# Luca96/carla-driving-rl-agent

Measured on AMD Instinct MI355X. Metric: PPO update-steps/sec (batch=256, 4x90x120x3 obs), higher is better.
Workload: dtype f32; 1 GPU; configs[1]: synthetic rollout buffer 256x4-frame 90x120x3 obs per GPU, full CARLANetwork fwd/bwd + PPO (re-sampled Beta, pathwise) / value loss + clip + Adam, fp32; per_gpu_batch=256, global_batch=256, parallelism=dp1, policy_loss=resampled (reference-faithful)

## Files before the change

### carla-driving-rl-agent_amd/csrc/gemm_pw_bwd.hip

```cpp
#include <stdlib.h>

#include "colreduce.h"

namespace cdrl {

typedef float f32x16 __attribute__((ext_vector_type(16)));
typedef __bf16 bf16x8 __attribute__((ext_vector_type(8)));
typedef __bf16 bf16x4 __attribute__((ext_vector_type(4)));
typedef uint32_t u32x2 __attribute__((ext_vector_type(2)));
typedef float f32x2 __attribute__((ext_vector_type(2)));

struct PwbArgs {
    View dz;
    int dz_shuffle;
    int act;
    const float* y;
    const float* stats;
    const float* coef;
    View a;
    const float* a_stats;
    const __bf16* Wp;
    int wp_ks;
    View da;
    float* qpart;
// ... 721 lines not shown
                    qacc[j] = __builtin_amdgcn_mfma_f32_32x32x16_bf16(a1, d1, qacc[j], 0, 0, 0);
                }
            }
        };
        if (t0 < t1) {
#pragma unroll
            for (int j = 0; j < 4; ++j) load_row(t0, j);
        }
        __syncthreads();
        for (int t = t0; t < t1; ++t) {
            store_tile(t);
            __syncthreads();
            compute_tile();
            __syncthreads();
        }
        float* qp = a.qpart + ((int64_t)g * a.nbpg + b) * KP * NP;
#pragma unroll
        for (int j = 0; j < NTW; ++j) {
            const int n = (qnt0 + j) * 32 + lrow;
#pragma unroll
            for (int r = 0; r < 16; ++r) {
                const int k = qkt * 32 + (r & 3) + 8 * (r >> 2) + 4 * lk;
                qp[k * NP + n] = qacc[j][r];
            }
        }
        __syncthreads();
        if (ANORM && a.spart) {
            __syncthreads();
            __syncthreads();
        }
    }
}

struct PwbReduceArgs {
    const float* qpart;
    const double* dbpart;
    const double* spart;
    const float* W;
    const float* a_stats;
    const float* a_gamma;
    const float* a_beta;
    float* dW;
    float* db;
    float* a_dgamma;
    float* a_dbeta;
    float* a_coef;
    const double* fin_tot;
    float* o_dgamma;
    float* o_dbeta;
    int N, K, KP, NP, G, Mg, nbpg;
    int wbf;
};

constexpr int PWB_RS = 8;
__global__ void __launch_bounds__(128 * PWB_RS) pwb_reduce_kernel(PwbReduceArgs a) {
    __shared__ double sq[PWB_RS][128];
    __shared__ double sd[PWB_RS][128];
    __shared__ double red[2][8][2];
    const int k = blockIdx.x, n = threadIdx.x & 127, sl = threadIdx.x >> 7;
    const int N = a.N, K = a.K, G = a.G;
    const bool on = n < N;
    const int nsl = PWB_RS / G > 0 ? PWB_RS / G : 1;
    const int per = (a.nbpg + nsl - 1) / nsl;
    for (int pair = sl; pair < G * nsl; pair += PWB_RS) {
        const int g = pair % G, s = pair / G;
        const int b0 = s * per, b1 = min(a.nbpg, b0 + per);
        double q = 0.0, d = 0.0;
        if (on) {
            const float* pq = a.qpart + ((int64_t)g * a.nbpg * a.KP + k) * a.NP + n;
            const double* pd = a.dbpart + (int64_t)g * a.nbpg * a.NP + n;
            int b = b0;
            const bool need_d = a.a_stats != nullptr || k == 0;
            for (; b + 32 <= b1; b += 32) {
                float v[32];
                double u[32];
#pragma unroll
                for (int i = 0; i < 32; ++i) {
                    v[i] = pq[(int64_t)(b + i) * a.KP * a.NP];
                    u[i] = need_d ? pd[(int64_t)(b + i) * a.NP] : 0.0;
                }
#pragma unroll
                for (int i = 0; i < 32; ++i) {
                    q += (double)v[i];
                    d += u[i];
                }
            }
            for (; b + 16 <= b1; b += 16) {
                float v[16];
                double u[16];
#pragma unroll
                for (int i = 0; i < 16; ++i) {
                    v[i] = pq[(int64_t)(b + i) * a.KP * a.NP];
                    u[i] = pd[(int64_t)(b + i) * a.NP];
                }
#pragma unroll
                for (int i = 0; i < 16; ++i) {
                    q += (double)v[i];
                    d += u[i];
                }
            }
            for (; b + 8 <= b1; b += 8) {
                float v[8];
                double u[8];
#pragma unroll
                for (int i = 0; i < 8; ++i) {
                    v[i] = pq[(int64_t)(b + i) * a.KP * a.NP];
                    u[i] = pd[(int64_t)(b + i) * a.NP];
                }
#pragma unroll
                for (int i = 0; i < 8; ++i) {
                    q += (double)v[i];
                    d += u[i];
                }
            }
            for (; b < b1; ++b) {
                q += (double)pq[(int64_t)b * a.KP * a.NP];
                d += pd[(int64_t)b * a.NP];
            }
        }
        sq[pair][n] = q;
        sd[pair][n] = d;
    }
    __syncthreads();
    const bool lead = sl == 0;
    float w = (on && lead) ? a.W[(int64_t)k * N + n] : 0.0f;
    if (a.wbf) w = (float)(__bf16)w;
    double qtot = 0.0, dbtot = 0.0;
    double s1[8], s2[8];
#pragma unroll
    for (int g = 0; g < 8; ++g) {
        s1[g] = s2[g] = 0.0;
        if (g < G && lead) {
            double q = sq[g][n], d = sd[g][n];
            for (int s = 1; s < nsl; ++s) {
                q += sq[s * G + g][n];
                d += sd[s * G + g][n];
            }
            qtot += q;
            dbtot += d;
            s1[g] = (double)w * d;
            s2[g] = (double)w * q;
        }
    }
    if (on && lead) {
        if (a.a_stats) a.dW[(int64_t)k * N + n] = (float)((double)a.a_gamma[k] * qtot + (double)a.a_beta[k] * dbtot);
        else a.dW[(int64_t)k * N + n] = (float)qtot;
        if (k == 0) a.db[n] = (float)dbtot;
        if (k == 0 && a.fin_tot) {
            double dg = 0.0, dbt = 0.0;
            for (int g = 0; g < G; ++g) {
                dbt += a.fin_tot[((int64_t)g * 2 + 0) * N + n];
                dg += a.fin_tot[((int64_t)g * 2 + 1) * N + n];
            }
            a.o_dgamma[n] = (float)dg;
            a.o_dbeta[n] = (float)dbt;
        }
    }
    if (!a.a_stats) return;
    const int lane = n & 63, wave = n >> 6;
#pragma unroll
    for (int g = 0; g < 8; ++g) {
        if (g >= G) break;
        double u1 = s1[g], u2 = s2[g];
#pragma unroll
        for (int o = 32; o > 0; o >>= 1) {
            u1 += __shfl_down(u1, o);
            u2 += __shfl_down(u2, o);
        }
        if (lane == 0 && lead) {
            red[0][g][wave] = u1;
            red[1][g][wave] = u2;
        }
    }
    __syncthreads();
    if (a.spart && (int)(threadIdx.x >> 6) < 2 * G) {
        const int pr = threadIdx.x >> 6, g = pr >> 1, q = pr & 1, l = threadIdx.x & 63;
        double u = 0.0;
        for (int b = l; b < a.nbpg; b += 64) u += a.spart[(((int64_t)g * a.nbpg + b) * 2 + q) * a.KP + k];
#pragma unroll
        for (int o = 32; o > 0; o >>= 1) u += __shfl_down(u, o);
        if (l == 0) {
            red[q][g][0] = u;
            red[q][g][1] = 0.0;
        }
    }
    __syncthreads();
    if (threadIdx.x == 0) {
        const int GK = G * K;
        const double cnt = (double)a.Mg;
        double dg = 0.0, dbt = 0.0;
        for (int g = 0; g < G; ++g) {
            const double u1 = red[0][g][0] + red[0][g][1], u2 = red[1][g][0] + red[1][g][1];
            dbt += u1;
            dg += u2;
            a.a_coef[0 * GK + g * K + k] = a.a_stats[2 * GK + g * K + k];
            a.a_coef[1 * GK + g * K + k] = (float)(u1 / cnt);
            a.a_coef[2 * GK + g * K + k] = (float)(u2 / cnt);
        }
        a.a_dgamma[k] = (float)dg;
        a.a_dbeta[k] = (float)dbt;
    }
}

static inline int pwb_pad(int c) { return c <= 64 ? 64 : 128; }

bool pw_bwd_fused_supported(View dz, View a, View da, int N, int K, int at) {
    if (N > 128 || K > 128 || N < 8 || K < 8 || (N & 1) || (K & 1)) return false;
    if (at && pwb_pad(N) != pwb_pad(K)) return false;
    if (pwb_pad(N) != pwb_pad(K) && !(pwb_pad(K) == 64 && pwb_pad(N) == 128)) return false;
    auto ok = [](View v) { return (v.ld % 2 == 0) && (v.coff % 2 == 0) && ((reinterpret_cast<uintptr_t>(v.p) & 7) == 0); };
    return ok(a) && ok(da) && (dz.ld % 2 == 0) && ((reinterpret_cast<uintptr_t>(dz.p) & 7) == 0);
}

int pw_bwd_fused_nbpg(int G, int Mg, int N, int K, int at) {
    const int bm = (pwb_pad(K) == 128 || pwb_pad(N) == 128) ? 32 : 64;
    const int tiles = cdiv(Mg, bm);
    int nb = 256 / G;
    if (at && tiles >= 6 * (512 / G)) nb = 512 / G;
    if (nb < 1) nb = 1;
    return nb > tiles ? tiles : nb;
}

int64_t pw_bwd_fused_qpart_elems(int G, int Mg, int N, int K, int at) {
    return (int64_t)G * pw_bwd_fused_nbpg(G, Mg, N, K, at) * pwb_pad(K) * pwb_pad(N);
}

int64_t pw_bwd_fused_dbpart_elems(int G, int Mg, int N, int K, int at) {
    return (int64_t)G * pw_bwd_fused_nbpg(G, Mg, N, K, at) * pwb_pad(N) * (at ? 3 : 1);
}

template <int KP, int NP, bool SHUF, bool ANORM, bool ACC>
static int pwb_launch(const PwbArgs& a, hipStream_t st) {
    constexpr int BM = (KP == 128 || NP == 128) ? 32 : 64;
    constexpr size_t lds = (size_t)(3 * BM * (NP + 8) + 3 * (NP + KP) * (BM + 8)) * 2 + (size_t)7 * NP * sizeof(float);
    auto kern = pwb_kernel<KP, NP, SHUF, ANORM, ACC>;
    static LdsAttrOnce attr;
    if (attr.need()) {
        CDRL_HIP(hipFuncSetAttribute(reinterpret_cast<const void*>(kern), hipFuncAttributeMaxDynamicSharedMemorySize, (int)lds));
        attr.mark();
    }
    hipLaunchKernelGGL(kern, dim3(a.G * a.nbpg), dim3(512), lds, st, a);
    CDRL_LAUNCH_CHECK();
    return 0;
}

template <int P, bool SHUF, bool ANORM, bool ACC>
static int pwb16_launch(const PwbArgs& a, hipStream_t st) {
    constexpr int BM = P == 128 ? 32 : 64;
    constexpr size_t lds = (size_t)(BM * (P + 8) + 2 * P * (BM + 8)) * 2 + (size_t)7 * P * sizeof(float) + (size_t)(P / 16) * 2 * 128 * 8 * 2;
    auto kern = pwb16_kernel<P, P, SHUF, ANORM, ACC>;
    static LdsAttrOnce attr;
    if (attr.need() && lds >= 64 * 1024) {
        CDRL_HIP(hipFuncSetAttribute(reinterpret_cast<const void*>(kern), hipFuncAttributeMaxDynamicSharedMemorySize, (int)lds));
// ... 62 lines not shown
        set_error("pw_bwd_fused: finalize-on-load needs the float32 form, fin_tot and fin_nb");
        return -1;
    }
    a.spart = (f.at && f.a_stats) ? f.dbpart + (int64_t)f.G * a.nbpg * pwb_pad(f.N) : nullptr;
    static const int dbg = cdrl_getenv("CDRL_DIAG_PWB") ? atoi(cdrl_getenv("CDRL_DIAG_PWB")) : 0;
    a.dbg = dbg;
    const bool anorm = f.a_stats != nullptr, acc = f.accumulate != 0, shuf = f.dz_shuffle != 0;
    if (f.at && pwb_pad(f.K) != pwb_pad(f.N)) {
        set_error("pw_bwd_fused: the bf16-storage form is instantiated for equal paddings only (N=%d K=%d)", f.N, f.K);
        return -1;
    }
    if (f.at) {
        if (pwb_pad(f.K) == 128) return shuf ? pwb16_launch2<128, true>(a, anorm, acc, st) : pwb16_launch2<128, false>(a, anorm, acc, st);
        return shuf ? pwb16_launch2<64, true>(a, anorm, acc, st) : pwb16_launch2<64, false>(a, anorm, acc, st);
    }
    if (pwb_pad(f.K) == 128) return shuf ? pwb_launch2<128, 128, true>(a, anorm, acc, st) : pwb_launch2<128, 128, false>(a, anorm, acc, st);
    if (pwb_pad(f.N) == 128) return shuf ? pwb_launch2<64, 128, true>(a, anorm, acc, st) : pwb_launch2<64, 128, false>(a, anorm, acc, st);
    return shuf ? pwb_launch2<64, 64, true>(a, anorm, acc, st) : pwb_launch2<64, 64, false>(a, anorm, acc, st);
}

int pw_bwd_fused_reduce(const PwBwdFused& f, hipStream_t st) {
    PwbReduceArgs r;
    r.qpart = f.qpart;
    r.dbpart = f.dbpart;
    r.W = f.W;
    r.a_stats = f.a_stats;
    r.a_gamma = f.a_gamma;
    r.a_beta = f.a_beta;
    r.dW = f.dW;
    r.db = f.db;
    r.a_dgamma = f.a_dgamma;
    r.a_dbeta = f.a_dbeta;
    r.a_coef = f.a_coef;
    r.N = f.N;
    r.K = f.K;
    r.KP = pwb_pad(f.K);
    r.NP = pwb_pad(f.N);
    r.G = f.G;
    r.Mg = f.Mg;
    r.nbpg = pw_bwd_fused_nbpg(f.G, f.Mg, f.N, f.K, f.at);
    r.wbf = f.at;
    r.fin_tot = (f.fin_part && !f.at) ? f.fin_tot : nullptr;
    r.o_dgamma = f.o_dgamma;
    r.o_dbeta = f.o_dbeta;
    if (r.fin_tot && (!f.o_dgamma || !f.o_dbeta)) {
        set_error("pw_bwd_fused_reduce: finalize-on-load needs the dgamma / dbeta outputs of the BatchNorm behind the conv");
        return -1;
    }
    r.spart = (f.at && f.a_stats) ? f.dbpart + (int64_t)f.G * r.nbpg * pwb_pad(f.N) : nullptr;
    if (f.a_stats && (!f.a_gamma || !f.a_beta || !f.a_dgamma || !f.a_dbeta || !f.a_coef)) {
        set_error("pw_bwd_fused_reduce: normalised input needs gamma / beta and the dgamma / dbeta / coef outputs");
        return -1;
    }
    hipLaunchKernelGGL(pwb_reduce_kernel, dim3(f.K), dim3(128 * PWB_RS), 0, st, r);
    CDRL_LAUNCH_CHECK();
    return 0;
}

}
```

### carla-driving-rl-agent_amd/csrc/gemm_pw_x3.hip

```cpp
#include <stdlib.h>

#include "cdrl_kernels.h"
#include "pack_bodies.h"

namespace cdrl {

typedef float f32x16 __attribute__((ext_vector_type(16)));
typedef __bf16 bf16x8 __attribute__((ext_vector_type(8)));
typedef __bf16 bf16x4 __attribute__((ext_vector_type(4)));

struct PwX3Args {
    View A;
    const float* pro_stats;
    const __bf16* Wp;
    const float* bias;
    View C;
    double* part;
    int N, K, G, Mg, nbpg;
};

__device__ __forceinline__ void split3(float x, __bf16& h1, __bf16& h2, __bf16& h3) {
    h1 = (__bf16)x;
    const float r1 = x - (float)h1;
    h2 = (__bf16)r1;
    h3 = (__bf16)(r1 - (float)h2);
}

template <int KP, int NT, bool PRO, bool EPI>
__global__ void __launch_bounds__(256, 2) pw_x3_kernel(PwX3Args a) {
    constexpr int WC = NT, WR = 4 / WC, BM = 32 * WR, KS = KP / 16;
    constexpr int LDA = KP + 8;
    constexpr int CPR = KP / 4;
    constexpr int NCH = BM * CPR / 256;
    __shared__ __attribute__((aligned(16))) __bf16 As[3][BM * LDA];
    __shared__ float pc[2][KP];
    __shared__ double red[2][4][32];
    const int tid = threadIdx.x, lane = tid & 63, wave = tid >> 6;
    const int wr = wave % WR, wc = wave / WR;
    const int lrow = lane & 31, lk = lane >> 5;
    const int g = blockIdx.x / a.nbpg, b = blockIdx.x % a.nbpg;
    const int K = a.K, N = a.N;
    const int64_t mbeg = (int64_t)g * a.Mg, mend = mbeg + a.Mg;
    const int tiles_g = (a.Mg + BM - 1) / BM;
    const int t0 = (int)((int64_t)b * tiles_g / a.nbpg), t1 = (int)((int64_t)(b + 1) * tiles_g / a.nbpg);
    const int n = wc * 32 + lrow;
    bf16x8 breg[3][KS];
#pragma unroll
    for (int p = 0; p < 3; ++p)
#pragma unroll
        for (int s = 0; s < KS; ++s)
            breg[p][s] = *reinterpret_cast<const bf16x8*>(a.Wp + (((int64_t)(p * KS + s) * 2 + lk) * 128 + n) * 8);
    const float bv = (a.bias && n < N) ? a.bias[n] : 0.0f;
    if (PRO) {
        const int GK = a.G * K;
        for (int k = tid; k < KP; k += 256) {
            pc[0][k] = k < K ? a.pro_stats[2 * GK + g * K + k] : 0.0f;
            pc[1][k] = k < K ? a.pro_stats[3 * GK + g * K + k] : 0.0f;
        }
        __syncthreads();
    }
    double s1 = 0.0, s2 = 0.0;
    typedef uint32_t u32x4_t __attribute__((ext_vector_type(4)));
    const uint32_t OOR = 0x80000000u;
    const int64_t Mtot = (int64_t)a.G * a.Mg;
    const __amdgpu_buffer_rsrc_t rsA = __builtin_amdgcn_make_buffer_rsrc(a.A.p, 0, (int)(Mtot * a.A.ld * 4), 0x00020000);
    u32x4_t ra[NCH];
    auto load_tile = [&](int t) {
        const int64_t m0 = mbeg + (int64_t)t * BM;
#pragma unroll
        for (int i = 0; i < NCH; ++i) {
            const int c = tid + 256 * i, r = c / CPR, k4 = 4 * (c % CPR);
            const bool ok = (m0 + r < mend) && (k4 < K);
            const uint32_t off = (uint32_t)(((m0 + r) * a.A.ld + a.A.coff + k4) * 4);
            ra[i] = __builtin_amdgcn_raw_buffer_load_b128(rsA, ok ? off : OOR, 0, 0);
        }
    };
    auto store_tile = [&]() {
        typedef float f32x2 __attribute__((ext_vector_type(2)));
        typedef __bf16 bf16x2 __attribute__((ext_vector_type(2)));
        typedef uint32_t u32x2_t __attribute__((ext_vector_type(2)));
        auto widen = [](uint32_t w) -> f32x2 { return f32x2{__uint_as_float(w << 16), __uint_as_float(w & 0xffff0000u)}; };
#pragma unroll
        for (int i = 0; i < NCH; ++i) {
            const int c = tid + 256 * i, r = c / CPR, k4 = 4 * (c % CPR);
            uint32_t hw[3][2];
#pragma unroll
            for (int h = 0; h < 2; ++h) {
                f32x2 x = f32x2{__uint_as_float(ra[i][2 * h]), __uint_as_float(ra[i][2 * h + 1])};
                if (k4 + 2 * h >= K) x[0] = 0.0f;
                if (k4 + 2 * h + 1 >= K) x[1] = 0.0f;
                if (PRO) {
                    const f32x2 sc = f32x2{pc[0][k4 + 2 * h], pc[0][k4 + 2 * h + 1]}, sh = f32x2{pc[1][k4 + 2 * h], pc[1][k4 + 2 * h + 1]};
                    x = __builtin_elementwise_fma(sc, x, sh);
                }
                hw[0][h] = __builtin_bit_cast(uint32_t, __builtin_convertvector(x, bf16x2));
                const f32x2 r1 = x - widen(hw[0][h]);
                hw[1][h] = __builtin_bit_cast(uint32_t, __builtin_convertvector(r1, bf16x2));
                hw[2][h] = __builtin_bit_cast(uint32_t, __builtin_convertvector(r1 - widen(hw[1][h]), bf16x2));
            }
#pragma unroll
            for (int p = 0; p < 3; ++p) *reinterpret_cast<u32x2_t*>(&As[p][r * LDA + k4]) = u32x2_t{hw[p][0], hw[p][1]};
        }
    };
    auto compute_tile = [&](int t) {
        f32x16 acc;
#pragma unroll
        for (int r = 0; r < 16; ++r) acc[r] = 0.0f;
        const int ao = (wr * 32 + lrow) * LDA + 8 * lk;
#pragma unroll
        for (int s = 0; s < KS; ++s) {
            const bf16x8 a1 = *reinterpret_cast<const bf16x8*>(&As[0][ao + 16 * s]);
            const bf16x8 a2 = *reinterpret_cast<const bf16x8*>(&As[1][ao + 16 * s]);
            const bf16x8 a3 = *reinterpret_cast<const bf16x8*>(&As[2][ao + 16 * s]);
            acc = __builtin_amdgcn_mfma_f32_32x32x16_bf16(a3, breg[0][s], acc, 0, 0, 0);
            acc = __builtin_amdgcn_mfma_f32_32x32x16_bf16(a1, breg[2][s], acc, 0, 0, 0);
            acc = __builtin_amdgcn_mfma_f32_32x32x16_bf16(a2, breg[1][s], acc, 0, 0, 0);
            acc = __builtin_amdgcn_mfma_f32_32x32x16_bf16(a2, breg[0][s], acc, 0, 0, 0);
            acc = __builtin_amdgcn_mfma_f32_32x32x16_bf16(a1, breg[1][s], acc, 0, 0, 0);
            acc = __builtin_amdgcn_mfma_f32_32x32x16_bf16(a1, breg[0][s], acc, 0, 0, 0);
        }
        if (n >= N) return;
        const int64_t m0 = mbeg + (int64_t)t * BM + wr * 32;
#pragma unroll
        for (int r = 0; r < 16; ++r) {
            const int64_t m = m0 + (r & 3) + 8 * (r >> 2) + 4 * lk;
            if (m < mend) {
                const float v = acc[r] + bv;
                if (EPI) {
                    s1 += (double)v;
                    s2 += (double)v * (double)v;
                }
                a.C.p[m * a.C.ld + a.C.coff + n] = v;
            }
        }
    };
    if (t0 < t1) load_tile(t0);
    for (int t = t0; t < t1; ++t) {
        store_tile();
        __syncthreads();
        if (t + 1 < t1) load_tile(t + 1);
        compute_tile(t);
        __syncthreads();
    }
    if (EPI && a.part) {
        const double f1 = s1 + __shfl_down(s1, 32), f2 = s2 + __shfl_down(s2, 32);
        if (lk == 0) {
            red[0][wave][lrow] = f1;
            red[1][wave][lrow] = f2;
        }
        __syncthreads();
        if (wr == 0 && lk == 0 && n < N) {
            double u1 = 0.0, u2 = 0.0;
#pragma unroll
            for (int w = 0; w < WR; ++w) {
                u1 += red[0][wc * WR + w][lrow];
                u2 += red[1][wc * WR + w][lrow];
            }
            double* p = a.part + ((int64_t)g * a.nbpg + b) * 2 * N;
            p[n] = u1;
            p[N + n] = u2;
        }
    }
}


template <bool PRO, bool EPI>
__global__ void __launch_bounds__(256, 2) pw_x3_wide_kernel(PwX3Args a) {
    constexpr int KP = 256, BM = 32, KS = KP / 16, LDA = KP + 8, CPR = KP / 4, NCH = BM * CPR / 256;
    __shared__ __attribute__((aligned(16))) __bf16 As[3][BM * LDA];
    __shared__ float pc[2][KP];
    const int tid = threadIdx.x, lane = tid & 63, wave = tid >> 6;
    const int lrow = lane & 31, lk = lane >> 5;
    const int g = blockIdx.x / a.nbpg, t = blockIdx.x % a.nbpg;
    const int K = a.K, N = a.N;
    const int64_t mbeg = (int64_t)g * a.Mg, mend = mbeg + a.Mg;
    const int64_t m0 = mbeg + (int64_t)t * BM;
    const int nl = wave * 32 + lrow, n = blockIdx.y * 128 + nl;
    typedef uint32_t u32x4_t __attribute__((ext_vector_type(4)));
    typedef float f32x2 __attribute__((ext_vector_type(2)));
    typedef __bf16 bf16x2 __attribute__((ext_vector_type(2)));
    typedef uint32_t u32x2_t __attribute__((ext_vector_type(2)));
    const uint32_t OOR = 0x80000000u;
    const int64_t Mtot = (int64_t)a.G * a.Mg;
    const __amdgpu_buffer_rsrc_t rsA = __builtin_amdgcn_make_buffer_rsrc(a.A.p, 0, (int)(Mtot * a.A.ld * 4), 0x00020000);
    u32x4_t ra[NCH];
#pragma unroll
    for (int i = 0; i < NCH; ++i) {
        const int c = tid + 256 * i, r = c / CPR, k4 = 4 * (c % CPR);
        const bool ok = (m0 + r < mend) && (k4 < K);
        const uint32_t off = (uint32_t)(((m0 + r) * a.A.ld + a.A.coff + k4) * 4);
        ra[i] = __builtin_amdgcn_raw_buffer_load_b128(rsA, ok ? off : OOR, 0, 0);
    }
    if (PRO) {
        const int GK = a.G * K;
        for (int k = tid; k < KP; k += 256) {
            pc[0][k] = k < K ? a.pro_stats[2 * GK + g * K + k] : 0.0f;
// ... 4 lines not shown
    constexpr int PF = 6;
    bf16x8 ring[PF][3];
    auto wload = [&](int s, bf16x8* dst) {
#pragma unroll
        for (int p = 0; p < 3; ++p) dst[p] = *reinterpret_cast<const bf16x8*>(wp + (int64_t)(p * KS + s) * 2 * 128 * 8);
    };
#pragma unroll
    for (int s = 0; s < PF; ++s) wload(s, ring[s]);
    const float bv = (a.bias && n < N) ? a.bias[n] : 0.0f;
    if (PRO) __syncthreads();
    {
        auto widen = [](uint32_t w) -> f32x2 { return f32x2{__uint_as_float(w << 16), __uint_as_float(w & 0xffff0000u)}; };
#pragma unroll
        for (int i = 0; i < NCH; ++i) {
            const int c = tid + 256 * i, r = c / CPR, k4 = 4 * (c % CPR);
            uint32_t hw[3][2];
#pragma unroll
            for (int h = 0; h < 2; ++h) {
                f32x2 x = f32x2{__uint_as_float(ra[i][2 * h]), __uint_as_float(ra[i][2 * h + 1])};
                if (k4 + 2 * h >= K) x[0] = 0.0f;
                if (k4 + 2 * h + 1 >= K) x[1] = 0.0f;
                if (PRO) {
                    const f32x2 sc = f32x2{pc[0][k4 + 2 * h], pc[0][k4 + 2 * h + 1]}, sh = f32x2{pc[1][k4 + 2 * h], pc[1][k4 + 2 * h + 1]};
                    x = __builtin_elementwise_fma(sc, x, sh);
                }
                hw[0][h] = __builtin_bit_cast(uint32_t, __builtin_convertvector(x, bf16x2));
                const f32x2 r1 = x - widen(hw[0][h]);
                hw[1][h] = __builtin_bit_cast(uint32_t, __builtin_convertvector(r1, bf16x2));
                hw[2][h] = __builtin_bit_cast(uint32_t, __builtin_convertvector(r1 - widen(hw[1][h]), bf16x2));
            }
#pragma unroll
            for (int p = 0; p < 3; ++p) *reinterpret_cast<u32x2_t*>(&As[p][r * LDA + k4]) = u32x2_t{hw[p][0], hw[p][1]};
        }
    }
    __syncthreads();
    f32x16 acc;
#pragma unroll
    for (int r = 0; r < 16; ++r) acc[r] = 0.0f;
    const int ao = lrow * LDA + 8 * lk;
#pragma unroll
    for (int s = 0; s < KS; ++s) {
        const bf16x8 a1 = *reinterpret_cast<const bf16x8*>(&As[0][ao + 16 * s]);
        const bf16x8 a2 = *reinterpret_cast<const bf16x8*>(&As[1][ao + 16 * s]);
        const bf16x8 a3 = *reinterpret_cast<const bf16x8*>(&As[2][ao + 16 * s]);
        const bf16x8 b1 = ring[s % PF][0], b2 = ring[s % PF][1], b3 = ring[s % PF][2];
        if (s + PF < KS) wload(s + PF, ring[s % PF]);
        acc = __builtin_amdgcn_mfma_f32_32x32x16_bf16(a3, b1, acc, 0, 0, 0);
        acc = __builtin_amdgcn_mfma_f32_32x32x16_bf16(a1, b3, acc, 0, 0, 0);
        acc = __builtin_amdgcn_mfma_f32_32x32x16_bf16(a2, b2, acc, 0, 0, 0);
        acc = __builtin_amdgcn_mfma_f32_32x32x16_bf16(a2, b1, acc, 0, 0, 0);
        acc = __builtin_amdgcn_mfma_f32_32x32x16_bf16(a1, b2, acc, 0, 0, 0);
        acc = __builtin_amdgcn_mfma_f32_32x32x16_bf16(a1, b1, acc, 0, 0, 0);
    }
    if (n >= N) return;
    double s1 = 0.0, s2 = 0.0;
#pragma unroll
    for (int r = 0; r < 16; ++r) {
        const int64_t m = m0 + (r & 3) + 8 * (r >> 2) + 4 * lk;
        if (m < mend) {
            const float v = acc[r] + bv;
            if (EPI) {
                s1 += (double)v;
                s2 += (double)v * (double)v;
            }
            a.C.p[m * a.C.ld + a.C.coff + n] = v;
        }
    }
    if (EPI && a.part) {
        const double f1 = s1 + __shfl_down(s1, 32), f2 = s2 + __shfl_down(s2, 32);
        if (lk == 0) {
            double* p = a.part + ((int64_t)g * a.nbpg + t) * 2 * N;
            p[n] = f1;
            p[N + n] = f2;
        }
    }
}


struct PwX3BwdArgs {
    View A;
    int a_shuffle, a_act;
    const float* a_y;
    const float* pro_stats;
    const float* pro_coef;
    double* part2;
    const __bf16* Wp;
    View C;
    const float* ey;
    const float* epi_stats;
    double* part;
    int N, K, G, Mg, nbpg;
};

template <bool SHUF, bool EPI, bool ACC>
__global__ void __launch_bounds__(256, 2) pw_x3_wide_bwd_kernel(PwX3BwdArgs a) {
    constexpr int KP = 256, BM = 32, KS = KP / 16, LDA = KP + 8, CPR = KP / 4, NCH = BM * CPR / 256;
    __shared__ __attribute__((aligned(16))) __bf16 As[3][BM * LDA];
    __shared__ float qc[7][KP];
    const int tid = threadIdx.x, lane = tid & 63, wave = tid >> 6;
    const int lrow = lane & 31, lk = lane >> 5;
    const int g = blockIdx.x / a.nbpg, t = blockIdx.x % a.nbpg;
    const int K = a.K, N = a.N;
    const int64_t mbeg = (int64_t)g * a.Mg, mend = mbeg + a.Mg;
    const int64_t m0 = mbeg + (int64_t)t * BM;
    const int nl = wave * 32 + lrow, n = blockIdx.y * 128 + nl;
    typedef uint32_t u32x4_t __attribute__((ext_vector_type(4)));
    typedef uint32_t u32x2_t __attribute__((ext_vector_type(2)));
    typedef float f32x2 __attribute__((ext_vector_type(2)));
    typedef __bf16 bf16x2 __attribute__((ext_vector_type(2)));
    const uint32_t OOR = 0x80000000u;
    const int64_t Mtot = (int64_t)a.G * a.Mg;
    const __amdgpu_buffer_rsrc_t rsA = __builtin_amdgcn_make_buffer_rsrc(a.A.p, 0, (int)(Mtot * a.A.ld * 4), 0x00020000);
    const __amdgpu_buffer_rsrc_t rsY = __builtin_amdgcn_make_buffer_rsrc(const_cast<float*>(a.a_y), 0, (int)(Mtot * K * 4), 0x00020000);
    const int k4 = 4 * (tid % CPR), r0 = tid / CPR;
    const bool kon = k4 < K;
    uint32_t voD0, voD1;
    if (SHUF) {
        voD0 = kon ? (uint32_t)shuffle_dst(a.A.coff + k4, a.a_shuffle) * 4u : OOR;
// ... 166 lines not shown

PwX3Pack pw_x3_pack_entry(const float* w, void* wp, int K, int N, int sbk, int sbn) {
    PwX3Pack e;
    e.w = w;
    e.wp = reinterpret_cast<__bf16*>(wp);
    e.K = K;
    e.N = N;
    e.sbk = sbk;
    e.sbn = sbn;
    e.kp = x3_wide(N, K) ? 256 : x3_kp(K);
    return e;
}

int pw_x3_pack_many(const PwX3Pack* tab_dev, int n, hipStream_t st) {
    if (n <= 0) return 0;
    hipLaunchKernelGGL(pw_x3_pack_many_kernel, dim3(8, n), dim3(256), 0, st, tab_dev);
    CDRL_LAUNCH_CHECK();
    return 0;
}

bool pw_x3_supported(View A, int N, int K) {
    if (K >= 4 && K <= 128 && N >= 1 && N <= 128 && K % 2 == 0 && A.ld % 2 == 0 && A.coff % 2 == 0 &&
        (reinterpret_cast<uintptr_t>(A.p) & 15) == 0)
        return true;
    return K >= 4 && K <= 256 && N >= 1 && N <= 256 && K % 4 == 0 && A.ld % 4 == 0 && A.coff % 4 == 0 &&
           (reinterpret_cast<uintptr_t>(A.p) & 15) == 0;
}

static constexpr int X3_OCC = 2;

int pw_x3_partial_rows(int G, int Mg, int N, int K) {
    if (x3_wide(N, K)) return cdiv(Mg, 32);
    const int bm = 32 * (4 / x3_nt(N)), tiles = cdiv(Mg, bm);
    int nb = 256 * X3_OCC / G;
    if (nb < 1) nb = 1;
    return nb > tiles ? tiles : nb;
}

template <int KP, int NT>
static void pw_x3_launch(const PwX3Args& a, bool pro, bool epi, hipStream_t st) {
    const dim3 grid(a.G * a.nbpg), block(256);
    if (pro && epi) hipLaunchKernelGGL((pw_x3_kernel<KP, NT, true, true>), grid, block, 0, st, a);
    else if (pro) hipLaunchKernelGGL((pw_x3_kernel<KP, NT, true, false>), grid, block, 0, st, a);
    else if (epi) hipLaunchKernelGGL((pw_x3_kernel<KP, NT, false, true>), grid, block, 0, st, a);
    else hipLaunchKernelGGL((pw_x3_kernel<KP, NT, false, false>), grid, block, 0, st, a);
}

int pw_x3(View A, const float* pro_stats, const void* Wp, const float* bias, View C, int G, int Mg, int N, int K, double* part,
          hipStream_t st, int nbpg) {
    if (!pw_x3_supported(A, N, K) || !Wp) {
        set_error("pw_x3: unsupported shape / alignment K=%d N=%d ld=%d coff=%d", K, N, A.ld, A.coff);
        return -1;
    }
    if ((int64_t)G * Mg * A.ld * 4 >= (int64_t)1 << 31) {
        set_error("pw_x3: operand of 2 GB or more");
        return -1;
    }
    PwX3Args a{A, pro_stats, reinterpret_cast<const __bf16*>(Wp), bias, C, part, N, K, G, Mg, nbpg > 0 ? nbpg : pw_x3_partial_rows(G, Mg, N, K)};
    const int kp = x3_kp(K), nt = x3_nt(N);
    const bool pro = pro_stats != nullptr, epi = part != nullptr;
    if (x3_wide(N, K)) {
        if (a.nbpg != cdiv(Mg, 32)) {
            set_error("pw_x3: the wide form writes one partial row per 32-row tile (%d), not %d", cdiv(Mg, 32), a.nbpg);
            return -1;
        }
        const dim3 grid(G * a.nbpg, cdiv(N, 128)), block(256);
        if (pro && epi) hipLaunchKernelGGL((pw_x3_wide_kernel<true, true>), grid, block, 0, st, a);
        else if (pro) hipLaunchKernelGGL((pw_x3_wide_kernel<true, false>), grid, block, 0, st, a);
        else if (epi) hipLaunchKernelGGL((pw_x3_wide_kernel<false, true>), grid, block, 0, st, a);
        else hipLaunchKernelGGL((pw_x3_wide_kernel<false, false>), grid, block, 0, st, a);
        CDRL_LAUNCH_CHECK();
        return 0;
    }
#define CDRL_X3(KPV, NTV) pw_x3_launch<KPV, NTV>(a, pro, epi, st)
    if (kp == 32) { if (nt == 1) CDRL_X3(32, 1); else if (nt == 2) CDRL_X3(32, 2); else CDRL_X3(32, 4); }
    else if (kp == 64) { if (nt == 1) CDRL_X3(64, 1); else if (nt == 2) CDRL_X3(64, 2); else CDRL_X3(64, 4); }
    else { if (nt == 1) CDRL_X3(128, 1); else if (nt == 2) CDRL_X3(128, 2); else CDRL_X3(128, 4); }
#undef CDRL_X3
    CDRL_LAUNCH_CHECK();
    return 0;
}


bool pw_x3_wide_bwd_supported(View dz, View C, int N, int K, int shuffle_ctot) {
    if (!(K > 128 || N > 128) || K > 256 || N > 256 || (K & 3)) return false;
    if ((reinterpret_cast<uintptr_t>(dz.p) & 15) || (dz.ld & 1)) return false;
    if (shuffle_ctot) return (dz.coff & 1) == 0 && ((shuffle_ctot >> 1) & 1) == 0;
    return (dz.ld & 3) == 0 && (dz.coff & 3) == 0;
}

int pw_x3_wide_bwd_rows(int Mg) { return cdiv(Mg, 32); }

int pw_x3_wide_bwd(View dz, const PwBnBwd& bb, const void* Wp, View C, int accumulate, int G, int Mg, int N, int K, const float* ey,
                   const float* epi_stats, double* part, hipStream_t st) {
    if (!pw_x3_wide_bwd_supported(dz, C, N, K, bb.shuffle_ctot) || !Wp || !bb.y || !bb.stats || !bb.coef) {
        set_error("pw_x3_wide_bwd: unsupported shape / alignment K=%d N=%d ld=%d coff=%d", K, N, dz.ld, dz.coff);
        return -1;
    }
    if ((ey != nullptr) && accumulate) {
        set_error("pw_x3_wide_bwd: the BatchNorm-sum epilogue and accumulation are not instantiated together");
        return -1;
    }
    const int64_t Mtot = (int64_t)G * Mg;
    if (Mtot * dz.ld * 4 >= (int64_t)1 << 31 || Mtot * K * 4 >= (int64_t)1 << 31 || Mtot * C.ld * 4 >= (int64_t)1 << 31) {
        set_error("pw_x3_wide_bwd: operand of 2 GB or more");
        return -1;
    }
// ... 35 lines not shown
```

Before: 79.58 update-steps/s.

## Split pointwise-backward reduce into plain and normalized-input kernels with narrower blocks

Replaces the single 1024-thread per-K reduce kernel with two specialized kernels. When the input is not normalized, a plain kernel tiles N in 32-column chunks across a 2D grid, so no threads sit idle for small N and more blocks run in parallel. When it is normalized, a templated kernel sized to the padded N uses 512 threads, spreads the per-group shuffle reductions and spart sums across slices, and parallelizes the final coefficient writes. The change is meant to cut idle lanes and serial tail work in this reduce, at the cost of more code paths and templated variants.

```diff
diff --git a/carla-driving-rl-agent_amd/csrc/gemm_pw_bwd.hip b/carla-driving-rl-agent_amd/csrc/gemm_pw_bwd.hip
--- a/carla-driving-rl-agent_amd/csrc/gemm_pw_bwd.hip
+++ b/carla-driving-rl-agent_amd/csrc/gemm_pw_bwd.hip
@@ -797,153 +797,192 @@
     int wbf;
 };
 
-constexpr int PWB_RS = 8;
-__global__ void __launch_bounds__(128 * PWB_RS) pwb_reduce_kernel(PwbReduceArgs a) {
-    __shared__ double sq[PWB_RS][128];
-    __shared__ double sd[PWB_RS][128];
-    __shared__ double red[2][8][2];
-    const int k = blockIdx.x, n = threadIdx.x & 127, sl = threadIdx.x >> 7;
-    const int N = a.N, K = a.K, G = a.G;
-    const bool on = n < N;
-    const int nsl = PWB_RS / G > 0 ? PWB_RS / G : 1;
+template <int B, int KR, bool D>
+__device__ __forceinline__ void pwb_red_batch(const float* pq, int64_t qs, int rs, const double* pd, int ds, double (&q)[KR], double& d) {
+    float v[KR][B];
+    double u[B];
+#pragma unroll
+    for (int i = 0; i < B; ++i) {
+#pragma unroll
+        for (int r = 0; r < KR; ++r) v[r][i] = pq[i * qs + r * rs];
+        if (D) u[i] = pd[(int64_t)i * ds];
+    }
+#pragma unroll
+    for (int i = 0; i < B; ++i) {
+#pragma unroll
+        for (int r = 0; r < KR; ++r) q[r] += (double)v[r][i];
+        if (D) d += u[i];
+    }
+}
+
+template <int KR, bool D>
+__device__ __forceinline__ void pwb_red_slice(const float* pq, int64_t qs, int rs, const double* pd, int ds, int b0, int b1, double (&q)[KR], double& d) {
+    int b = b0;
+    for (; b + 32 <= b1; b += 32) pwb_red_batch<32, KR, D>(pq + b * qs, qs, rs, pd + (int64_t)b * ds, ds, q, d);
+    for (; b + 16 <= b1; b += 16) pwb_red_batch<16, KR, D>(pq + b * qs, qs, rs, pd + (int64_t)b * ds, ds, q, d);
+    for (; b + 8 <= b1; b += 8) pwb_red_batch<8, KR, D>(pq + b * qs, qs, rs, pd + (int64_t)b * ds, ds, q, d);
+    for (; b < b1; ++b) pwb_red_batch<1, KR, D>(pq + b * qs, qs, rs, pd + (int64_t)b * ds, ds, q, d);
+}
+
+constexpr int PWB_PAIRS = 8;
+
+__device__ __forceinline__ void pwb_red_col_outputs(const PwbReduceArgs& a, int n, double dbtot) {
+    a.db[n] = (float)dbtot;
+    if (a.fin_tot) {
+        double dg = 0.0, dbt = 0.0;
+        for (int g = 0; g < a.G; ++g) {
+            dbt += a.fin_tot[((int64_t)g * 2 + 0) * a.N + n];
+            dg += a.fin_tot[((int64_t)g * 2 + 1) * a.N + n];
+        }
+        a.o_dgamma[n] = (float)dg;
+        a.o_dbeta[n] = (float)dbt;
+    }
+}
+
+constexpr int PWB_PN = 32;
+__global__ void __launch_bounds__(PWB_PN * PWB_PAIRS) pwb_reduce_plain_kernel(PwbReduceArgs a) {
+    __shared__ double sq[PWB_PAIRS][PWB_PN];
+    __shared__ double sd[PWB_PAIRS][PWB_PN];
+    const int k = blockIdx.x, nl = threadIdx.x % PWB_PN, n = blockIdx.y * PWB_PN + nl, sl = threadIdx.x / PWB_PN;
+    const int G = a.G;
+    const bool on = n < a.N;
+    const int nsl = PWB_PAIRS / G > 0 ? PWB_PAIRS / G : 1;
     const int per = (a.nbpg + nsl - 1) / nsl;
-    for (int pair = sl; pair < G * nsl; pair += PWB_RS) {
+    const int64_t qs = (int64_t)a.KP * a.NP;
+    for (int pair = sl; pair < G * nsl; pair += PWB_PAIRS) {
         const int g = pair % G, s = pair / G;
         const int b0 = s * per, b1 = min(a.nbpg, b0 + per);
-        double q = 0.0, d = 0.0;
+        double q[1] = {0.0}, d = 0.0;
         if (on) {
             const float* pq = a.qpart + ((int64_t)g * a.nbpg * a.KP + k) * a.NP + n;
             const double* pd = a.dbpart + (int64_t)g * a.nbpg * a.NP + n;
-            int b = b0;
-            const bool need_d = a.a_stats != nullptr || k == 0;
-            for (; b + 32 <= b1; b += 32) {
-                float v[32];
-                double u[32];
-#pragma unroll
-                for (int i = 0; i < 32; ++i) {
-                    v[i] = pq[(int64_t)(b + i) * a.KP * a.NP];
-                    u[i] = need_d ? pd[(int64_t)(b + i) * a.NP] : 0.0;
-                }
-#pragma unroll
-                for (int i = 0; i < 32; ++i) {
-                    q += (double)v[i];
-                    d += u[i];
-                }
-            }
-            for (; b + 16 <= b1; b += 16) {
-                float v[16];
-                double u[16];
-#pragma unroll
-                for (int i = 0; i < 16; ++i) {
-                    v[i] = pq[(int64_t)(b + i) * a.KP * a.NP];
-                    u[i] = pd[(int64_t)(b + i) * a.NP];
-                }
-#pragma unroll
-                for (int i = 0; i < 16; ++i) {
-                    q += (double)v[i];
-                    d += u[i];
-                }
-            }
-            for (; b + 8 <= b1; b += 8) {
-                float v[8];
-                double u[8];
-#pragma unroll
-                for (int i = 0; i < 8; ++i) {
-                    v[i] = pq[(int64_t)(b + i) * a.KP * a.NP];
-                    u[i] = pd[(int64_t)(b + i) * a.NP];
-                }
-#pragma unroll
-                for (int i = 0; i < 8; ++i) {
-                    q += (double)v[i];
-                    d += u[i];
-                }
-            }
-            for (; b < b1; ++b) {
-                q += (double)pq[(int64_t)b * a.KP * a.NP];
-                d += pd[(int64_t)b * a.NP];
-            }
-        }
-        sq[pair][n] = q;
+            if (k == 0) pwb_red_slice<1, true>(pq, qs, 0, pd, a.NP, b0, b1, q, d);
+            else pwb_red_slice<1, false>(pq, qs, 0, pd, a.NP, b0, b1, q, d);
+        }
+        sq[pair][nl] = q[0];
+        sd[pair][nl] = d;
+    }
+    __syncthreads();
+    if (sl != 0 || !on) return;
+    double qtot = 0.0, dbtot = 0.0;
+    for (int g = 0; g < G; ++g) {
+        double q = sq[g][nl], d = sd[g][nl];
+        for (int s = 1; s < nsl; ++s) {
+            q += sq[s * G + g][nl];
+            d += sd[s * G + g][nl];
+        }
+        qtot += q;
+        dbtot += d;
+    }
+    a.dW[(int64_t)k * a.N + n] = (float)qtot;
+    if (k == 0) pwb_red_col_outputs(a, n, dbtot);
+}
+
+template <int NT, int KR>
+__global__ void __launch_bounds__(512) pwb_reduce_anorm_kernel(PwbReduceArgs a) {
+    constexpr int SL = 512 / NT;
+    constexpr int WPR = NT / 64;
+    __shared__ double sq[KR][PWB_PAIRS][NT];
+    __shared__ double sd[PWB_PAIRS][NT];
+    __shared__ double red[KR][2][8][2];
+    const int k0 = blockIdx.x * KR, n = threadIdx.x % NT, sl = threadIdx.x / NT;
+    const int N = a.N, K = a.K, G = a.G;
+    const bool on = n < N;
+    const int nsl = PWB_PAIRS / G > 0 ? PWB_PAIRS / G : 1;
+    const int per = (a.nbpg + nsl - 1) / nsl;
+    const int64_t qs = (int64_t)a.KP * a.NP;
+    for (int pair = sl; pair < G * nsl; pair += SL) {
+        const int g = pair % G, s = pair / G;
+        const int b0 = s * per, b1 = min(a.nbpg, b0 + per);
+        double q[KR], d = 0.0;
+#pragma unroll
+        for (int r = 0; r < KR; ++r) q[r] = 0.0;
+        if (on) {
+            const float* pq = a.qpart + ((int64_t)g * a.nbpg * a.KP + k0) * a.NP + n;
+            const double* pd = a.dbpart + (int64_t)g * a.nbpg * a.NP + n;
+            pwb_red_slice<KR, true>(pq, qs, a.NP, pd, a.NP, b0, b1, q, d);
+        }
+#pragma unroll
+        for (int r = 0; r < KR; ++r) sq[r][pair][n] = q[r];
         sd[pair][n] = d;
     }
     __syncthreads();
-    const bool lead = sl == 0;
-    float w = (on && lead) ? a.W[(int64_t)k * N + n] : 0.0f;
-    if (a.wbf) w = (float)(__bf16)w;
-    double qtot = 0.0, dbtot = 0.0;
-    double s1[8], s2[8];
-#pragma unroll
-    for (int g = 0; g < 8; ++g) {
-        s1[g] = s2[g] = 0.0;
-        if (g < G && lead) {
-            double q = sq[g][n], d = sd[g][n];
-            for (int s = 1; s < nsl; ++s) {
-                q += sq[s * G + g][n];
-                d += sd[s * G + g][n];
-            }
-            qtot += q;
-            dbtot += d;
-            s1[g] = (double)w * d;
-            s2[g] = (double)w * q;
-        }
-    }
-    if (on && lead) {
-        if (a.a_stats) a.dW[(int64_t)k * N + n] = (float)((double)a.a_gamma[k] * qtot + (double)a.a_beta[k] * dbtot);
-        else a.dW[(int64_t)k * N + n] = (float)qtot;
-        if (k == 0) a.db[n] = (float)dbtot;
-        if (k == 0 && a.fin_tot) {
-            double dg = 0.0, dbt = 0.0;
-            for (int g = 0; g < G; ++g) {
-                dbt += a.fin_tot[((int64_t)g * 2 + 0) * N + n];
-                dg += a.fin_tot[((int64_t)g * 2 + 1) * N + n];
-            }
-            a.o_dgamma[n] = (float)dg;
-            a.o_dbeta[n] = (float)dbt;
-        }
-    }
-    if (!a.a_stats) return;
-    const int lane = n & 63, wave = n >> 6;
-#pragma unroll
-    for (int g = 0; g < 8; ++g) {
-        if (g >= G) break;
-        double u1 = s1[g], u2 = s2[g];
+    const int lane = threadIdx.x & 63, half = (threadIdx.x / 64) % WPR;
+    for (int c = sl; c < KR * G; c += SL) {
+        const int r = c / G, g = c % G, k = k0 + r;
+        if (k >= K) continue;
+        float w = on ? a.W[(int64_t)k * N + n] : 0.0f;
+        if (a.wbf) w = (float)(__bf16)w;
+        double q = sq[r][g][n], d = sd[g][n];
+        for (int s = 1; s < nsl; ++s) {
+            q += sq[r][s * G + g][n];
+            d += sd[s * G + g][n];
+        }
+        double u1 = (double)w * d, u2 = (double)w * q;
 #pragma unroll
         for (int o = 32; o > 0; o >>= 1) {
             u1 += __shfl_down(u1, o);
             u2 += __shfl_down(u2, o);
         }
-        if (lane == 0 && lead) {
-            red[0][g][wave] = u1;
-            red[1][g][wave] = u2;
-        }
+        if (lane == 0) {
+            red[r][0][g][half] = u1;
+            red[r][1][g][half] = u2;
+            if (WPR == 1) red[r][0][g][1] = red[r][1][g][1] = 0.0;
+        }
+    }
+    for (int r = SL - 1 - sl; r < KR; r += SL) {
+        const int k = k0 + r;
+        if (k >= K || !on) continue;
+        double qtot = 0.0, dbtot = 0.0;
+        for (int g = 0; g < G; ++g) {
+            double q = sq[r][g][n], d = sd[g][n];
+            for (int s = 1; s < nsl; ++s) {
+                q += sq[r][s * G + g][n];
+                d += sd[s * G + g][n];
+            }
+            qtot += q;
+            dbtot += d;
+        }
+        a.dW[(int64_t)k * N + n] = (float)((double)a.a_gamma[k] * qtot + (double)a.a_beta[k] * dbtot);
+        if (k == 0) pwb_red_col_outputs(a, n, dbtot);
     }
     __syncthreads();
-    if (a.spart && (int)(threadIdx.x >> 6) < 2 * G) {
-        const int pr = threadIdx.x >> 6, g = pr >> 1, q = pr & 1, l = threadIdx.x & 63;
-        double u = 0.0;
-        for (int b = l; b < a.nbpg; b += 64) u += a.spart[(((int64_t)g * a.nbpg + b) * 2 + q) * a.KP + k];
-#pragma unroll
-        for (int o = 32; o > 0; o >>= 1) u += __shfl_down(u, o);
-        if (l == 0) {
-            red[q][g][0] = u;
-            red[q][g][1] = 0.0;
-        }
-    }
-    __syncthreads();
-    if (threadIdx.x == 0) {
-        const int GK = G * K;
-        const double cnt = (double)a.Mg;
-        double dg = 0.0, dbt = 0.0;
-        for (int g = 0; g < G; ++g) {
-            const double u1 = red[0][g][0] + red[0][g][1], u2 = red[1][g][0] + red[1][g][1];
-            dbt += u1;
-            dg += u2;
+    if (a.spart) {
+        for (int pr = threadIdx.x >> 6; pr < KR * 2 * G; pr += 8) {
+            const int r = pr / (2 * G), g = (pr % (2 * G)) >> 1, q = pr & 1, k = k0 + r;
+            if (k >= K) continue;
+            double u = 0.0;
+            for (int b = lane; b < a.nbpg; b += 64) u += a.spart[(((int64_t)g * a.nbpg + b) * 2 + q) * a.KP + k];
+#pragma unroll
+            for (int o = 32; o > 0; o >>= 1) u += __shfl_down(u, o);
+            if (lane == 0) {
+                red[r][q][g][0] = u;
+                red[r][q][g][1] = 0.0;
+            }
+        }
+        __syncthreads();
+    }
+    const int GK = G * K;
+    if ((int)threadIdx.x < KR * G) {
+        const int r = threadIdx.x / G, g = threadIdx.x % G, k = k0 + r;
+        if (k < K) {
+            const double cnt = (double)a.Mg;
+            const double u1 = red[r][0][g][0] + red[r][0][g][1], u2 = red[r][1][g][0] + red[r][1][g][1];
             a.a_coef[0 * GK + g * K + k] = a.a_stats[2 * GK + g * K + k];
             a.a_coef[1 * GK + g * K + k] = (float)(u1 / cnt);
             a.a_coef[2 * GK + g * K + k] = (float)(u2 / cnt);
         }
-        a.a_dgamma[k] = (float)dg;
-        a.a_dbeta[k] = (float)dbt;
+    } else if (threadIdx.x >= 64 && (int)threadIdx.x < 64 + KR) {
+        const int r = threadIdx.x - 64, k = k0 + r;
+        if (k < K) {
+            double dg = 0.0, dbt = 0.0;
+            for (int g = 0; g < G; ++g) {
+                dbt += red[r][0][g][0] + red[r][0][g][1];
+                dg += red[r][1][g][0] + red[r][1][g][1];
+            }
+            a.a_dgamma[k] = (float)dg;
+            a.a_dbeta[k] = (float)dbt;
+        }
     }
 }
 
@@ -1112,7 +1151,9 @@
         set_error("pw_bwd_fused_reduce: normalised input needs gamma / beta and the dgamma / dbeta / coef outputs");
         return -1;
     }
-    hipLaunchKernelGGL(pwb_reduce_kernel, dim3(f.K), dim3(128 * PWB_RS), 0, st, r);
+    if (!f.a_stats) hipLaunchKernelGGL(pwb_reduce_plain_kernel, dim3(f.K, cdiv(f.N, PWB_PN)), dim3(PWB_PN * PWB_PAIRS), 0, st, r);
+    else if (r.NP == 128) hipLaunchKernelGGL((pwb_reduce_anorm_kernel<128, 1>), dim3(f.K), dim3(512), 0, st, r);
+    else hipLaunchKernelGGL((pwb_reduce_anorm_kernel<64, 1>), dim3(f.K), dim3(512), 0, st, r);
     CDRL_LAUNCH_CHECK();
     return 0;
 }
```

Result: no change. 80.14 update-steps/s (median of 5 runs) (+0.7%).

## Double-buffer LDS tiles and deepen prefetch in pointwise x3 GEMM

Applied to the files above, without the earlier changes.

Restructures the pointwise bf16x3 GEMM main loop so the split of the next tile into LDS overlaps with the current tile's MFMA work. It uses two LDS buffers when they fit and keeps two register tiles in flight with loads issued three tiles ahead. Prologue scale/shift stats now live in registers instead of LDS, and output stores go through buffer stores with out-of-range masking instead of branches. This adds register pressure and LDS use, which may lower occupancy, and it makes the loop schedule more complex.

```diff
diff --git a/carla-driving-rl-agent_amd/csrc/gemm_pw_x3.hip b/carla-driving-rl-agent_amd/csrc/gemm_pw_x3.hip
--- a/carla-driving-rl-agent_amd/csrc/gemm_pw_x3.hip
+++ b/carla-driving-rl-agent_amd/csrc/gemm_pw_x3.hip
@@ -32,10 +32,11 @@
     constexpr int LDA = KP + 8;
     constexpr int CPR = KP / 4;
     constexpr int NCH = BM * CPR / 256;
-    __shared__ __attribute__((aligned(16))) __bf16 As[3][BM * LDA];
-    __shared__ float pc[2][KP];
+    constexpr int NBUF = (2 * 3 * BM * LDA * 2 <= 56 * 1024) ? 2 : 1;
+    static_assert(256 % CPR == 0, "a thread's chunks all cover the same four columns");
+    __shared__ __attribute__((aligned(16))) __bf16 As[NBUF][3][BM * LDA];
     __shared__ double red[2][4][32];
-    const int tid = threadIdx.x, lane = tid & 63, wave = tid >> 6;
+    const int tid = threadIdx.x, lane = tid & 63, wave = __builtin_amdgcn_readfirstlane(tid >> 6);
     const int wr = wave % WR, wc = wave / WR;
     const int lrow = lane & 31, lk = lane >> 5;
     const int g = blockIdx.x / a.nbpg, b = blockIdx.x % a.nbpg;
@@ -44,6 +45,38 @@
     const int tiles_g = (a.Mg + BM - 1) / BM;
     const int t0 = (int)((int64_t)b * tiles_g / a.nbpg), t1 = (int)((int64_t)(b + 1) * tiles_g / a.nbpg);
     const int n = wc * 32 + lrow;
+    typedef uint32_t u32x4_t __attribute__((ext_vector_type(4)));
+    typedef float f32x2 __attribute__((ext_vector_type(2)));
+    typedef __bf16 bf16x2 __attribute__((ext_vector_type(2)));
+    typedef uint32_t u32x2_t __attribute__((ext_vector_type(2)));
+    const uint32_t OOR = 0x80000000u;
+    const int64_t Mtot = (int64_t)a.G * a.Mg;
+    const __amdgpu_buffer_rsrc_t rsA = __builtin_amdgcn_make_buffer_rsrc(a.A.p, 0, (int)(Mtot * a.A.ld * 4), 0x00020000);
+    const int k4 = 4 * (tid % CPR), r0 = tid / CPR;
+    u32x4_t ra[2][NCH];
+    auto load_tile = [&](int t, u32x4_t* dst) {
+        const int64_t m0 = mbeg + (int64_t)t * BM;
+#pragma unroll
+        for (int i = 0; i < NCH; ++i) {
+            const int r = r0 + (256 / CPR) * i;
+            const bool ok = (t < t1) && (m0 + r < mend) && (k4 < K);
+            const uint32_t off = (uint32_t)(((m0 + r) * a.A.ld + a.A.coff + k4) * 4);
+            dst[i] = __builtin_amdgcn_raw_buffer_load_b128(rsA, ok ? off : OOR, 0, 0);
+        }
+    };
+    f32x2 psc[2], psh[2];
+    if (PRO) {
+        const int GK = a.G * K;
+        const __amdgpu_buffer_rsrc_t rsP = __builtin_amdgcn_make_buffer_rsrc(const_cast<float*>(a.pro_stats), 0, 4 * GK * 4, 0x00020000);
+#pragma unroll
+        for (int e = 0; e < 4; ++e) {
+            const uint32_t oe = k4 + e < K ? (uint32_t)(g * K + k4 + e) * 4u : OOR;
+            const float sc = __uint_as_float(__builtin_amdgcn_raw_buffer_load_b32(rsP, oe, (uint32_t)(2 * GK) * 4u, 0));
+            const float sh = __uint_as_float(__builtin_amdgcn_raw_buffer_load_b32(rsP, oe, (uint32_t)(3 * GK) * 4u, 0));
+            psc[e >> 1][e & 1] = sc;
+            psh[e >> 1][e & 1] = sh;
+        }
+    }
     bf16x8 breg[3][KS];
 #pragma unroll
     for (int p = 0; p < 3; ++p)
@@ -51,67 +84,43 @@
         for (int s = 0; s < KS; ++s)
             breg[p][s] = *reinterpret_cast<const bf16x8*>(a.Wp + (((int64_t)(p * KS + s) * 2 + lk) * 128 + n) * 8);
     const float bv = (a.bias && n < N) ? a.bias[n] : 0.0f;
-    if (PRO) {
-        const int GK = a.G * K;
-        for (int k = tid; k < KP; k += 256) {
-            pc[0][k] = k < K ? a.pro_stats[2 * GK + g * K + k] : 0.0f;
-            pc[1][k] = k < K ? a.pro_stats[3 * GK + g * K + k] : 0.0f;
-        }
-        __syncthreads();
-    }
+    load_tile(t0, ra[0]);
+    load_tile(t0 + 1, ra[1]);
     double s1 = 0.0, s2 = 0.0;
-    typedef uint32_t u32x4_t __attribute__((ext_vector_type(4)));
-    const uint32_t OOR = 0x80000000u;
-    const int64_t Mtot = (int64_t)a.G * a.Mg;
-    const __amdgpu_buffer_rsrc_t rsA = __builtin_amdgcn_make_buffer_rsrc(a.A.p, 0, (int)(Mtot * a.A.ld * 4), 0x00020000);
-    u32x4_t ra[NCH];
-    auto load_tile = [&](int t) {
-        const int64_t m0 = mbeg + (int64_t)t * BM;
+    auto split_tile = [&](const u32x4_t* src, int buf) {
+        auto widen = [](uint32_t w) -> f32x2 { return f32x2{__uint_as_float(w << 16), __uint_as_float(w & 0xffff0000u)}; };
 #pragma unroll
         for (int i = 0; i < NCH; ++i) {
-            const int c = tid + 256 * i, r = c / CPR, k4 = 4 * (c % CPR);
-            const bool ok = (m0 + r < mend) && (k4 < K);
-            const uint32_t off = (uint32_t)(((m0 + r) * a.A.ld + a.A.coff + k4) * 4);
-            ra[i] = __builtin_amdgcn_raw_buffer_load_b128(rsA, ok ? off : OOR, 0, 0);
-        }
-    };
-    auto store_tile = [&]() {
-        typedef float f32x2 __attribute__((ext_vector_type(2)));
-        typedef __bf16 bf16x2 __attribute__((ext_vector_type(2)));
-        typedef uint32_t u32x2_t __attribute__((ext_vector_type(2)));
-        auto widen = [](uint32_t w) -> f32x2 { return f32x2{__uint_as_float(w << 16), __uint_as_float(w & 0xffff0000u)}; };
-#pragma unroll
-        for (int i = 0; i < NCH; ++i) {
-            const int c = tid + 256 * i, r = c / CPR, k4 = 4 * (c % CPR);
+            const int r = r0 + (256 / CPR) * i;
             uint32_t hw[3][2];
 #pragma unroll
             for (int h = 0; h < 2; ++h) {
-                f32x2 x = f32x2{__uint_as_float(ra[i][2 * h]), __uint_as_float(ra[i][2 * h + 1])};
+                f32x2 x = f32x2{__uint_as_float(src[i][2 * h]), __uint_as_float(src[i][2 * h + 1])};
                 if (k4 + 2 * h >= K) x[0] = 0.0f;
                 if (k4 + 2 * h + 1 >= K) x[1] = 0.0f;
-                if (PRO) {
-                    const f32x2 sc = f32x2{pc[0][k4 + 2 * h], pc[0][k4 + 2 * h + 1]}, sh = f32x2{pc[1][k4 + 2 * h], pc[1][k4 + 2 * h + 1]};
-                    x = __builtin_elementwise_fma(sc, x, sh);
-                }
+                if (PRO) x = __builtin_elementwise_fma(psc[h], x, psh[h]);
                 hw[0][h] = __builtin_bit_cast(uint32_t, __builtin_convertvector(x, bf16x2));
                 const f32x2 r1 = x - widen(hw[0][h]);
                 hw[1][h] = __builtin_bit_cast(uint32_t, __builtin_convertvector(r1, bf16x2));
                 hw[2][h] = __builtin_bit_cast(uint32_t, __builtin_convertvector(r1 - widen(hw[1][h]), bf16x2));
             }
 #pragma unroll
-            for (int p = 0; p < 3; ++p) *reinterpret_cast<u32x2_t*>(&As[p][r * LDA + k4]) = u32x2_t{hw[p][0], hw[p][1]};
+            for (int p = 0; p < 3; ++p) *reinterpret_cast<u32x2_t*>(&As[buf][p][r * LDA + k4]) = u32x2_t{hw[p][0], hw[p][1]};
         }
     };
-    auto compute_tile = [&](int t) {
+    const __amdgpu_buffer_rsrc_t rsC = __builtin_amdgcn_make_buffer_rsrc(a.C.p, 0, (int)(Mtot * a.C.ld * 4), 0x00020000);
+    const uint32_t rowC = (uint32_t)a.C.ld * 4u;
+    const uint32_t voC = n < N ? (uint32_t)((4 * lk) * a.C.ld + a.C.coff + n) * 4u : OOR;
+    auto step = [&](int t, u32x4_t* next, int buf) {
         f32x16 acc;
 #pragma unroll
         for (int r = 0; r < 16; ++r) acc[r] = 0.0f;
         const int ao = (wr * 32 + lrow) * LDA + 8 * lk;
 #pragma unroll
         for (int s = 0; s < KS; ++s) {
-            const bf16x8 a1 = *reinterpret_cast<const bf16x8*>(&As[0][ao + 16 * s]);
-            const bf16x8 a2 = *reinterpret_cast<const bf16x8*>(&As[1][ao + 16 * s]);
-            const bf16x8 a3 = *reinterpret_cast<const bf16x8*>(&As[2][ao + 16 * s]);
+            const bf16x8 a1 = *reinterpret_cast<const bf16x8*>(&As[buf][0][ao + 16 * s]);
+            const bf16x8 a2 = *reinterpret_cast<const bf16x8*>(&As[buf][1][ao + 16 * s]);
+            const bf16x8 a3 = *reinterpret_cast<const bf16x8*>(&As[buf][2][ao + 16 * s]);
             acc = __builtin_amdgcn_mfma_f32_32x32x16_bf16(a3, breg[0][s], acc, 0, 0, 0);
             acc = __builtin_amdgcn_mfma_f32_32x32x16_bf16(a1, breg[2][s], acc, 0, 0, 0);
             acc = __builtin_amdgcn_mfma_f32_32x32x16_bf16(a2, breg[1][s], acc, 0, 0, 0);
@@ -119,29 +128,45 @@
             acc = __builtin_amdgcn_mfma_f32_32x32x16_bf16(a1, breg[1][s], acc, 0, 0, 0);
             acc = __builtin_amdgcn_mfma_f32_32x32x16_bf16(a1, breg[0][s], acc, 0, 0, 0);
         }
-        if (n >= N) return;
+        __builtin_amdgcn_sched_barrier(0);
+        if (NBUF == 1) __syncthreads();
+        split_tile(next, NBUF == 2 ? buf ^ 1 : 0);
+        __builtin_amdgcn_sched_barrier(0);
         const int64_t m0 = mbeg + (int64_t)t * BM + wr * 32;
+        const uint32_t mu = (uint32_t)m0;
+        const int left = (int)(mend - m0) - 4 * lk;
+        float v[16];
 #pragma unroll
         for (int r = 0; r < 16; ++r) {
-            const int64_t m = m0 + (r & 3) + 8 * (r >> 2) + 4 * lk;
-            if (m < mend) {
-                const float v = acc[r] + bv;
-                if (EPI) {
-                    s1 += (double)v;
-                    s2 += (double)v * (double)v;
+            const int rr = (r & 3) + 8 * (r >> 2);
+            v[r] = acc[r] + bv;
+            __builtin_amdgcn_raw_buffer_store_b32(__float_as_uint(v[r]), rsC, voC | (rr < left ? 0u : OOR), (mu + (uint32_t)rr) * rowC, 0);
+        }
+        load_tile(t + 3, next);
+        __builtin_amdgcn_sched_barrier(0);
+        if (EPI && n < N) {
+#pragma unroll
+            for (int r = 0; r < 16; ++r) {
+                const int rr = (r & 3) + 8 * (r >> 2);
+                if (rr < left) {
+                    s1 += (double)v[r];
+                    s2 += (double)v[r] * (double)v[r];
                 }
-                a.C.p[m * a.C.ld + a.C.coff + n] = v;
             }
         }
+        __syncthreads();
     };
-    if (t0 < t1) load_tile(t0);
-    for (int t = t0; t < t1; ++t) {
-        store_tile();
-        __syncthreads();
-        if (t + 1 < t1) load_tile(t + 1);
-        compute_tile(t);
-        __syncthreads();
-    }
+    split_tile(ra[0], 0);
+    load_tile(t0 + 2, ra[0]);
+    __syncthreads();
+    int t = t0;
+    for (; t + 1 < t1; t += 2) {
+        step(t, ra[1], 0);
+        step(t + 1, ra[0], NBUF == 2 ? 1 : 0);
+    }
+    if (t < t1) step(t, ra[1], 0);
+#pragma unroll
+    for (int i = 0; i < NCH; ++i) asm volatile("" ::"v"(ra[0][i]), "v"(ra[1][i]));
     if (EPI && a.part) {
         const double f1 = s1 + __shfl_down(s1, 32), f2 = s2 + __shfl_down(s2, 32);
         if (lk == 0) {
@@ -252,18 +277,27 @@
         acc = __builtin_amdgcn_mfma_f32_32x32x16_bf16(a1, b2, acc, 0, 0, 0);
         acc = __builtin_amdgcn_mfma_f32_32x32x16_bf16(a1, b1, acc, 0, 0, 0);
     }
+    const __amdgpu_buffer_rsrc_t rsC = __builtin_amdgcn_make_buffer_rsrc(a.C.p, 0, (int)(Mtot * a.C.ld * 4), 0x00020000);
+    const uint32_t rowC = (uint32_t)a.C.ld * 4u, mu = (uint32_t)m0;
+    const uint32_t voC = n < N ? (uint32_t)((4 * lk) * a.C.ld + a.C.coff + n) * 4u : OOR;
+    const int left = (int)(mend - m0) - 4 * lk;
+    float v[16];
+#pragma unroll
+    for (int r = 0; r < 16; ++r) {
+        const int rr = (r & 3) + 8 * (r >> 2);
+        v[r] = acc[r] + bv;
+        __builtin_amdgcn_raw_buffer_store_b32(__float_as_uint(v[r]), rsC, voC | (rr < left ? 0u : OOR), (mu + (uint32_t)rr) * rowC, 0);
+    }
     if (n >= N) return;
     double s1 = 0.0, s2 = 0.0;
-#pragma unroll
-    for (int r = 0; r < 16; ++r) {
-        const int64_t m = m0 + (r & 3) + 8 * (r >> 2) + 4 * lk;
-        if (m < mend) {
-            const float v = acc[r] + bv;
-            if (EPI) {
-                s1 += (double)v;
-                s2 += (double)v * (double)v;
+    if (EPI) {
+#pragma unroll
+        for (int r = 0; r < 16; ++r) {
+            const int rr = (r & 3) + 8 * (r >> 2);
+            if (rr < left) {
+                s1 += (double)v[r];
+                s2 += (double)v[r] * (double)v[r];
             }
-            a.C.p[m * a.C.ld + a.C.coff + n] = v;
         }
     }
     if (EPI && a.part) {
@@ -536,7 +570,7 @@
         set_error("pw_x3: unsupported shape / alignment K=%d N=%d ld=%d coff=%d", K, N, A.ld, A.coff);
         return -1;
     }
-    if ((int64_t)G * Mg * A.ld * 4 >= (int64_t)1 << 31) {
+    if ((int64_t)G * Mg * A.ld * 4 >= (int64_t)1 << 31 || (int64_t)G * Mg * C.ld * 4 >= (int64_t)1 << 31) {
         set_error("pw_x3: operand of 2 GB or more");
         return -1;
     }
```

New measurement: 78.98 update-steps/s before, 79.58 update-steps/s after (median of 4 runs). About the same (+0.8%).
